# UMich-CURLY/SE3ET

Hardware: AMD Instinct MI355X
Metric: point-cloud pairs/sec (fwd), SE3ET-E 5k-pt pairs (higher is better)
Workload: dtype f32

## Files before the change

se3et_amd/csrc/kpconv_mfma.hip:

```cpp
#include "common.h"
#include "kpconv_sums.h"

namespace {

using namespace kpsum;
using f16x8 = __attribute__((ext_vector_type(8))) _Float16;
using f32x16 = __attribute__((ext_vector_type(16))) float;
using u32x4 = __attribute__((ext_vector_type(4))) unsigned;
using f32x4 = __attribute__((ext_vector_type(4))) float;

#ifndef SE3_KPCONV_STAMP
#define SE3_KPCONV_STAMP(step_, slot_)
#endif
#ifndef SE3_DIAG_WEIGHT_STEP
#define SE3_DIAG_WEIGHT_STEP(gs_, ksp_) (gs_)
#endif

constexpr int kTile4 = kTileB / 16;
constexpr int kHeaderB = 256;

__global__ void kpconv_wmax_kernel(const float* __restrict__ W, int64_t n, unsigned* __restrict__ hdr) {
  float m = 0.f;
  for (int64_t i = (int64_t)blockIdx.x * blockDim.x + threadIdx.x; i < n; i += (int64_t)gridDim.x * blockDim.x) m = fmaxf(m, fabsf(W[i]));
  m = se3_wave_max(m);
  if (se3_lane() == 0) atomicMax(hdr + 1, __float_as_uint(m));
}

__device__ __forceinline__ float weight_scale(unsigned max_bits) {
  const int e = (int)((max_bits >> 23) & 0xff);
  if (e == 0 || e == 0xff) return 1.f;
  return __uint_as_float((unsigned)(127 + 12 - (e - 127)) << 23);
}

__global__ void kpconv_split_weights_f16_kernel(const float* __restrict__ W, int Cin, int Cout, unsigned* __restrict__ hdr,
                                                uint4* __restrict__ Wf) {
  const int NCT = Cout / 32;
  const int64_t frag = blockIdx.x;
  const int ct = (int)(frag % NCT), st = (int)((frag / NCT) % kSteps), cc = (int)(frag / ((int64_t)NCT * kSteps));
  const int lane = threadIdx.x, n = ct * 32 + (lane & 31), u = 2 * st + (lane >> 5);
  const float scale = weight_scale(hdr[1]);
  if (frag == 0 && lane == 0) reinterpret_cast<float*>(hdr)[0] = 1.f / scale;
  f16x8 hi, lo;
#pragma unroll
  for (int j = 0; j < 8; j++) {
    const float w = W[((int64_t)u * Cin + cc * kCC + j) * Cout + n] * scale;
    hi[j] = (_Float16)w;
    lo[j] = (_Float16)(w - (float)hi[j]);
  }
  uint4* dst = Wf + frag * 2 * 64 + lane;
  dst[0] = __builtin_bit_cast(uint4, hi);
  dst[64] = __builtin_bit_cast(uint4, lo);
}

__device__ __forceinline__ int row_point(int i) { return ((i >> 3) << 2) + (i & 3); }
__device__ __forceinline__ int row_rsel(int i) { return (0x96 >> (i >> 2)) & 1; }

template <int NCW, int KS>
__global__ __launch_bounds__(64 * NCW * KS) void kpconv_mfma_kernel(const u32x4* __restrict__ H, const u32x4* __restrict__ Wf,
                                                                    const float* __restrict__ hdr, int64_t P, int64_t tiles, int Cin,
                                                                    int Cout, float* __restrict__ out) {
  constexpr int kThreads = 64 * NCW * KS;
  constexpr int kPF = (kTile4 + kThreads - 1) / kThreads;
  constexpr int kSPW = kSteps / KS;
  static_assert(kSteps % KS == 0, "K split must divide the 18 K16-steps of a chunk");
  extern __shared__ __align__(16) unsigned char lds[];
  unsigned* tab = reinterpret_cast<unsigned*>(lds + kTileB);
  const int tid = threadIdx.x, lane = tid & 63, wave = tid >> 6, cw = wave % NCW, ksp = wave / NCW;
  const int64_t tile = blockIdx.x, p0 = tile * kTP;
  const int NCT = Cout / 32, ct = blockIdx.y * NCW + cw;
  for (int e = tid; e < kSteps * 4; e += kThreads) {
    const int h = e & 1, rsel = (e >> 1) & 1, st = e >> 2;
    const int u = 2 * st + h, s = u / kA, t = u % kA;
    unsigned v = 0;
    for (int rt = 0; rt < 3; rt++) {
      const int r = 2 * rt + rsel;
      v |= (unsigned)run_of(kOrb.id[s][r], kOrb.anchor[t][r]) << (8 * rt);
    }
    tab[e] = v;
  }
  const int i32 = lane & 31, h = lane >> 5;
  const int a_base = row_point(i32) * kRowB;
  const int tab_lane = row_rsel(i32) * 2 + h;
  f32x16 acc[3];
#pragma unroll
  for (int rt = 0; rt < 3; rt++)
#pragma unroll
    for (int v = 0; v < 16; v++) acc[rt][v] = 0.f;
  const int chunks = Cin / kCC;
  u32x4 pf[kPF];
  {
    const u32x4* src = H + tile * kTile4;
#pragma unroll
    for (int i = 0; i < kPF; i++) pf[i] = src[min(tid + i * kThreads, kTile4 - 1)];
  }
  const u32x4* wbase = Wf + (int64_t)ct * 2 * 64 + lane;
  const int64_t wstep = (int64_t)NCT * 2 * 64;
  u32x4 bn0 = wbase[(int64_t)ksp * wstep], bn1 = wbase[(int64_t)ksp * wstep + 64];
  const int64_t last_step = (int64_t)chunks * kSteps - KS + ksp;
  for (int cc = 0; cc < chunks; cc++) {
    __syncthreads();
#pragma unroll
    for (int i = 0; i < kPF; i++)
      if (tid + i * kThreads < kTile4) reinterpret_cast<u32x4*>(lds)[tid + i * kThreads] = pf[i];
    {
      const int cn = cc + 1 < chunks ? cc + 1 : cc;
      const u32x4* src = H + ((int64_t)cn * tiles + tile) * kTile4;
#pragma unroll
      for (int i = 0; i < kPF; i++) pf[i] = src[min(tid + i * kThreads, kTile4 - 1)];
// ... 208 lines not shown
}

constexpr int kStageRow[4] = {0, 392, 836, 1228};
constexpr int kStageDw = 1228 + 384;
template <bool EXT>
__global__ __launch_bounds__(256) void kpconv_orbit_gather_kernel(const float* __restrict__ x, const float* __restrict__ hwt,
                                                                   const int* __restrict__ nbr, const int* __restrict__ cnt, int NNp,
                                                                   int64_t tiles, int Cin, unsigned char* __restrict__ Hs) {
  __shared__ __align__(16) unsigned stage[4][kStageDw];
  const int lane = threadIdx.x & 63, wave = threadIdx.x >> 6, g = lane >> 4, c16 = lane & 15, odd = c16 & 1, half = c16 >> 3;
  const int64_t p = blockIdx.x;
  const int T = blockIdx.y * 4 + wave, chunks = Cin / kCC;
  if (2 * T >= chunks) return;
  const bool has2 = 2 * T + 1 < chunks;
  const unsigned rowlen = (unsigned)(kA * Cin), col = (unsigned)(T * 16 + (has2 || half == 0 ? c16 : c16 - 8));
  const int nv = cnt[p];
  const int* nbrow = nbr + p * NNp;
  const float* hwrow = hwt + p * NNp * 16;
  f32x4 acc[kA];
#pragma unroll
  for (int a = 0; a < kA; a++) acc[a] = f32x4{0.f, 0.f, 0.f, 0.f};
  constexpr int S = EXT ? 40 : 32;
  for (int rd = 0; S * rd < nv; rd++) {
    int nbv[kGN + (EXT ? kGX : 0)];
    GatherOps<EXT> q;
    gather_request_rows<EXT>(nbrow, rd, g, nbv);
    gather_request_ops<EXT, false>(x, hwrow, NNp, rd, g, c16, nbv, rowlen, col, Cin, nv, q);
    gather_multiply<EXT>(q, nv > S * rd + 32, acc);
  }
  unsigned word[kA][4];
  gather_split(acc, odd, word);
  unsigned* st = stage[wave];
  const int cpair = (c16 & 7) >> 1;
#pragma unroll
  for (int a = 0; a < kA; a++)
#pragma unroll
    for (int r = 0; r < 4; r++) st[kStageRow[half * 2 + odd] + (a * 16 + 4 * g + r) * 4 + cpair] = word[a][r];
  for (int e = lane; e < 4 * 96; e += 64) {
    const int row = e / 96, q4 = e - row * 96, hf = row >> 1, piece = row & 1;
    if (hf == 1 && !has2) continue;
    unsigned char* dst = Hs + ((int64_t)(2 * T + hf) * tiles + (p >> 4)) * kTileB + (size_t)piece * kPieceB + (size_t)(p & 15) * kRowB;
    reinterpret_cast<u32x4*>(dst)[q4] = *reinterpret_cast<const u32x4*>(st + kStageRow[row] + q4 * 4);
  }
}

template <int NCW, int KS, int CT, bool EXT, bool BLK>
__global__ __launch_bounds__(64 * (NCW * KS + 8)) void kpconv_fused_kernel(
    const float* __restrict__ x, const float* __restrict__ hwt, const int* __restrict__ nbr, const int* __restrict__ cnt, int NNp,
    const u32x4* __restrict__ Wf, const float* __restrict__ hdr, int64_t P, int Cin, int Cout, float* __restrict__ out,
    float* __restrict__ split_part, int* __restrict__ split_count, const float* __restrict__ x_amax) {
  constexpr int NC = NCW * KS;
  const float xs = x_split_scale(x_amax);
  constexpr int NPW = 8;
  constexpr int kSPW = kSteps / KS;
  static_assert(kSteps % KS == 0, "K split must divide the 18 K16-steps of a chunk");
  extern __shared__ __align__(16) unsigned char lds[];
  unsigned* tab = reinterpret_cast<unsigned*>(lds + 3 * kTileB);
  const int tid = threadIdx.x, lane = tid & 63;
  const int wave = __builtin_amdgcn_readfirstlane(tid >> 6);
  const int64_t tile = blockIdx.x, p0 = tile * kTP;
  const int chunks = Cin / kCC / (int)gridDim.z, chunk0 = blockIdx.z * chunks, pairs = (chunks + 1) / 2;
  for (int e = tid; e < kSteps * 4; e += 64 * (NC + NPW)) {
    const int h = e & 1, rsel = (e >> 1) & 1, st = e >> 2;
    const int u = 2 * st + h, s = u / kA, t = u % kA;
    unsigned v = 0;
    for (int rt = 0; rt < 3; rt++) {
      const int r = 2 * rt + rsel;
      v |= (unsigned)run_of(kOrb.id[s][r], kOrb.anchor[t][r]) << (8 * rt);
    }
    tab[e] = v;
  }
  const int steps_total = chunks + 2;
  if (wave >= NC) {
    const int pw = wave - NC;
    const int g = lane >> 4, c16 = lane & 15, odd = c16 & 1, half = c16 >> 3, cpair = (c16 & 7) >> 1;
    const unsigned rowlen = (unsigned)(kA * Cin);
    const int dst0 = odd * kPieceB + g * 64 + cpair * 4;
    unsigned held[kA][4];
#pragma unroll
    for (int a = 0; a < kA; a++)
#pragma unroll
      for (int r = 0; r < 4; r++) held[a][r] = 0u;
    constexpr int S = EXT ? 40 : 32;
    GatherOps<EXT> ops;
    int nv_cur = 0;
    const int64_t plast = P - 1;
    auto point_of = [&](int u) { return p0 + pw + NPW * (u & 1); };
    auto col_of = [&](int u) {
      const int T = u >> 1;
      return (unsigned)(chunk0 * kCC + T * 16 + ((2 * T + 1 < chunks || half == 0) ? c16 : c16 - 8));
    };
    {
      const int64_t p = point_of(0), pc = p < P ? p : plast;
      int nbv[kGN + (EXT ? kGX : 0)];
      gather_request_rows<EXT>(nbr + pc * NNp, 0, g, nbv);
      nv_cur = p < P ? cnt[pc] : 0;
      gather_request_ops<EXT, BLK>(x, hwt + pc * NNp * 16, NNp, 0, g, c16, nbv, rowlen, col_of(0), Cin, __builtin_amdgcn_readfirstlane(nv_cur), ops);
    }
    for (int u = 0; u < steps_total; u++) {
      SE3_KPCONV_STAMP(u, 0)
      if (u < 2 * pairs) {
        const int T = u >> 1, second = u & 1;
        const int i = pw + NPW * second;
        const int64_t p = p0 + i, pc = p < P ? p : plast;
        const bool has2 = 2 * T + 1 < chunks;
        unsigned char* img_a = lds + ((2 * T) % 3) * kTileB;
        unsigned char* img_b = lds + ((2 * T + 1) % 3) * kTileB;
        if (second && half == 1 && has2) {
// ... 5 lines not shown
        }
        const bool more = u + 1 < 2 * pairs;
        const int64_t pn = point_of(u + 1), pnc = pn < P ? pn : plast;
        int nbn[kGN + (EXT ? kGX : 0)];
        gather_request_rows<EXT>(nbr + pnc * NNp, 0, g, nbn);
        const int nv_next = (more && pn < P) ? cnt[pnc] : 0;
        SE3_KPCONV_STAMP(u, 1)
        f32x4 acc[kA];
#pragma unroll
        for (int a = 0; a < kA; a++) acc[a] = f32x4{0.f, 0.f, 0.f, 0.f};
        const int nv = __builtin_amdgcn_readfirstlane(nv_cur);
        SE3_KPCONV_STAMP(u, 5)
        if (nv > 0) gather_multiply<EXT>(ops, nv > 32, acc, xs);
        SE3_KPCONV_STAMP(u, 6)
        for (int rd = 1; S * rd < nv; rd++) {
          int nbv[kGN + (EXT ? kGX : 0)];
          GatherOps<EXT> q;
          gather_request_rows<EXT>(nbr + pc * NNp, rd, g, nbv);
          gather_request_ops<EXT, BLK>(x, hwt + pc * NNp * 16, NNp, rd, g, c16, nbv, rowlen, col_of(u), Cin, nv, q);
          gather_multiply<EXT>(q, nv > S * rd + 32, acc, xs);
        }
        SE3_KPCONV_STAMP(u, 7)
        gather_request_ops<EXT, BLK>(x, hwt + pnc * NNp * 16, NNp, 0, g, c16, nbn, rowlen, col_of(more ? u + 1 : u), Cin,
                                __builtin_amdgcn_readfirstlane(nv_next), ops);
        nv_cur = nv_next;
        SE3_KPCONV_STAMP(u, 2)
        unsigned word[kA][4];
        gather_split(acc, odd, word);
        unsigned char* dst = (half ? img_b : img_a) + i * kRowB + dst0;
        if (half == 0 || (second && has2)) {
#pragma unroll
          for (int a = 0; a < kA; a++)
#pragma unroll
            for (int r = 0; r < 4; r++) *reinterpret_cast<unsigned*>(dst + (a * 16 + r) * 16) = word[a][r];
        }
#pragma unroll
        for (int a = 0; a < kA; a++)
#pragma unroll
          for (int r = 0; r < 4; r++) held[a][r] = word[a][r];
      }
      SE3_KPCONV_STAMP(u, 3)
      if (u + 1 < steps_total) __syncthreads();
      SE3_KPCONV_STAMP(u, 4)
    }
    if (KS > 1) {
      __syncthreads();
      __syncthreads();
    }
    return;
  }
  const int cw = wave % NCW, ksp = wave / NCW;
  const int NCT = Cout / 32, ct0 = (blockIdx.y * NCW + cw) * CT;
  const int i32 = lane & 31, h = lane >> 5;
  const int a_base = row_point(i32) * kRowB;
  const int tab_lane = row_rsel(i32) * 2 + h;
  f32x16 acc[CT][3];
#pragma unroll
  for (int n = 0; n < CT; n++)
#pragma unroll
    for (int rt = 0; rt < 3; rt++)
#pragma unroll
      for (int v = 0; v < 16; v++) acc[n][rt][v] = 0.f;
  constexpr int BD = (CT == 2 && KS > 1) ? 2 : (CT == 1 ? 6 : 3);
  constexpr int U = BD == 2 ? 2 : 6;
  static_assert(kSPW % U == 0, "K16-steps per wave and chunk must be a multiple of the unroll");
  const int64_t wstep = (int64_t)NCT * 2 * 64;
  const u32x4* wbase = Wf + (int64_t)chunk0 * kSteps * wstep + (int64_t)ct0 * 2 * 64 + lane;
  const int64_t last_step = (int64_t)chunks * kSteps - KS + ksp;
  u32x4 bq[BD][CT][2];
#pragma unroll
  for (int j = 0; j < BD; j++) {
    int64_t gs = ksp + j * KS;
    gs = gs < last_step ? gs : last_step;
#pragma unroll
    for (int n = 0; n < CT; n++) {
      bq[j][n][0] = wbase[gs * wstep + n * 128];
      bq[j][n][1] = wbase[gs * wstep + n * 128 + 64];
    }
  }
  __syncthreads();
  __syncthreads();
  for (int cc = 0; cc < chunks; cc++) {
    const unsigned char* img = lds + (cc % 3) * kTileB;
    SE3_KPCONV_STAMP(cc + 2, 0)
    f16x8 av[2][3][2];
    {
      const unsigned runs = tab[ksp * 4 + tab_lane];
#pragma unroll
      for (int rt = 0; rt < 3; rt++) {
        const int off = a_base + (int)((runs >> (8 * rt)) & 0xff) * 16;
        av[0][rt][0] = *reinterpret_cast<const f16x8*>(img + off);
        av[0][rt][1] = *reinterpret_cast<const f16x8*>(img + off + kPieceB);
      }
    }
#pragma unroll 1
    for (int q0 = 0; q0 < kSPW; q0 += U) {
#pragma unroll
      for (int j = 0; j < U; j++) {
        constexpr int kDummy = 0;
        const int ja = j & 1, jb = j % BD;
        const int st = ksp + (q0 + j) * KS;
        {
          const int sn = st + KS < kSteps ? st + KS : st;
          const unsigned runs = tab[sn * 4 + tab_lane];
#pragma unroll
          for (int rt = 0; rt < 3; rt++) {
            const int off = a_base + (int)((runs >> (8 * rt)) & 0xff) * 16;
            av[ja ^ 1][rt][0] = *reinterpret_cast<const f16x8*>(img + off);
            av[ja ^ 1][rt][1] = *reinterpret_cast<const f16x8*>(img + off + kPieceB);
          }
          if constexpr (CT == 1) __builtin_amdgcn_sched_barrier(0);
        }
#pragma unroll
        for (int n = 0; n < CT; n++) {
          const f16x8 b0 = __builtin_bit_cast(f16x8, bq[jb][n][0]);
#pragma unroll
          for (int rt = 0; rt < 3; rt++) acc[n][rt] = __builtin_amdgcn_mfma_f32_32x32x16_f16(av[ja][rt][1], b0, acc[n][rt], 0, 0, 0);
        }
#pragma unroll
        for (int n = 0; n < CT; n++) {
          const f16x8 b1 = __builtin_bit_cast(f16x8, bq[jb][n][1]);
#pragma unroll
          for (int rt = 0; rt < 3; rt++) acc[n][rt] = __builtin_amdgcn_mfma_f32_32x32x16_f16(av[ja][rt][0], b1, acc[n][rt], 0, 0, 0);
        }
#pragma unroll
        for (int n = 0; n < CT; n++) {
          const f16x8 b0 = __builtin_bit_cast(f16x8, bq[jb][n][0]);
#pragma unroll
          for (int rt = 0; rt < 3; rt++) acc[n][rt] = __builtin_amdgcn_mfma_f32_32x32x16_f16(av[ja][rt][0], b0, acc[n][rt], 0, 0, 0);
        }
        {
          int64_t gs = (int64_t)cc * kSteps + st + BD * KS;
          gs = gs < last_step ? gs : last_step;
          gs = SE3_DIAG_WEIGHT_STEP(gs, ksp);
#pragma unroll
          for (int n = 0; n < CT; n++) {
            bq[jb][n][0] = wbase[gs * wstep + n * 128];
            bq[jb][n][1] = wbase[gs * wstep + n * 128 + 64];
          }
        }
        (void)kDummy;
      }
    }
    SE3_KPCONV_STAMP(cc + 2, 3)
    if (cc + 1 < chunks) __syncthreads();
    SE3_KPCONV_STAMP(cc + 2, 4)
  }
  if (KS > 1) {
    __syncthreads();
    float* red = reinterpret_cast<float*>(lds);
    if (ksp > 0) {
#pragma unroll
      for (int n = 0; n < CT; n++)
#pragma unroll
        for (int rt = 0; rt < 3; rt++)
#pragma unroll
          for (int v = 0; v < 16; v++) red[((((ksp - 1) * NCW + cw) * CT + n) * 48 + rt * 16 + v) * 64 + lane] = acc[n][rt][v];
    }
    __syncthreads();
    if (ksp > 0) return;
#pragma unroll 1
    for (int k = 1; k < KS; k++)
#pragma unroll
      for (int n = 0; n < CT; n++)
#pragma unroll
        for (int rt = 0; rt < 3; rt++)
#pragma unroll
          for (int v = 0; v < 16; v++) acc[n][rt][v] += red[((((k - 1) * NCW + cw) * CT + n) * 48 + rt * 16 + v) * 64 + lane];
  }
  const float inv_scale = hdr[0] / xs;
  const int row_b = Cout * 4;
  const int rows_here = (int)(P - p0 < kTP ? P - p0 : kTP);
  int voff[CT][2];
#pragma unroll
  for (int n = 0; n < CT; n++) {
    voff[n][0] = ((ct0 + n) * 32 + i32) * 4 + h * row_b;
    voff[n][1] = ((ct0 + n) * 32 + i32) * 4 + (1 - h) * row_b;
  }
  constexpr int kAgent = 16;
#pragma unroll
  for (int n = 0; n < CT; n++)
#pragma unroll
    for (int rt = 0; rt < 3; rt++) acc[n][rt] *= inv_scale;
  if (gridDim.z > 1) {
    const int64_t rows_all = (int64_t)gridDim.x * kTP * kA;
    {
      const __amdgpu_buffer_rsrc_t prs =
          __builtin_amdgcn_make_buffer_rsrc(split_part + (blockIdx.z * rows_all + p0 * kA) * Cout, 0, kTP * kA * row_b, 0x00020000);
#pragma unroll
      for (int n = 0; n < CT; n++)
#pragma unroll
        for (int rt = 0; rt < 3; rt++)
#pragma unroll
          for (int v = 0; v < 16; v++) {
            const float val = acc[n][rt][v];
            __builtin_amdgcn_raw_buffer_store_b32(__builtin_bit_cast(unsigned, val), prs, voff[n][(0x6 >> (v >> 2)) & 1],
// ... 258 lines not shown
```

se3et_amd/csrc/kpconv_union.hip:

```cpp
#include "common.h"
#include "kpconv_sums.h"

namespace {

using namespace kpsum;
using f16x8 = __attribute__((ext_vector_type(8))) _Float16;
using f32x16 = __attribute__((ext_vector_type(16))) float;
using u32x4 = __attribute__((ext_vector_type(4))) unsigned;
using f32x4 = __attribute__((ext_vector_type(4))) float;

constexpr int kHeaderB = 256;
#ifndef SE3_UCAP
#define SE3_UCAP 128
#endif
constexpr int kUCap = SE3_UCAP;
constexpr int kKSM = kUCap / 32;
constexpr int kBFragB = 1024;
constexpr int kBImgB = 2 * 3 * kKSM * kBFragB;
constexpr int kScrRow = kUCap + 4;
constexpr int kMaxSub = 16;

__device__ __forceinline__ int row_point(int i) { return ((i >> 3) << 2) + (i & 3); }
__device__ __forceinline__ int row_rsel(int i) { return (0x96 >> (i >> 2)) & 1; }

struct PlanViews {
  int* order;
  int* nsub;
  int4* desc;
  int* urow;
  unsigned char* loc;
};
__host__ __device__ inline size_t align16(size_t v) { return (v + 15) & ~(size_t)15; }
inline PlanViews plan_views(void* plan, int64_t G, int NNp) {
  unsigned char* p = static_cast<unsigned char*>(plan);
  PlanViews v;
  v.order = reinterpret_cast<int*>(p);
  p += align16((size_t)G * 16 * sizeof(int));
  v.nsub = reinterpret_cast<int*>(p);
  p += align16((size_t)G * sizeof(int));
  v.desc = reinterpret_cast<int4*>(p);
  p += (size_t)G * kMaxSub * sizeof(int4);
  v.urow = reinterpret_cast<int*>(p);
  p += align16((size_t)G * 16 * NNp * sizeof(int));
  v.loc = p;
  return v;
}
inline size_t plan_bytes(int64_t G, int NNp) {
  return align16((size_t)G * 16 * sizeof(int)) + align16((size_t)G * sizeof(int)) + (size_t)G * kMaxSub * sizeof(int4) +
         align16((size_t)G * 16 * NNp * sizeof(int)) + align16((size_t)G * 16 * NNp) + 256;
}

struct NeighborTable {
  const float* hwt;
  const int *nbr, *cnt;
  int NNp;
};
NeighborTable table_views(const void* table, int64_t P, int NN) {
  NeighborTable t;
  t.NNp = NN <= 32 ? 32 : (NN + 39) / 40 * 40;
  t.hwt = static_cast<const float*>(table);
  t.nbr = reinterpret_cast<const int*>(t.hwt + (size_t)P * t.NNp * 16);
  t.cnt = t.nbr + (size_t)P * t.NNp;
  return t;
}

__global__ __launch_bounds__(64) void kpconv_union_plan_kernel(const int* __restrict__ nbr, const int* __restrict__ cnt, int NNp,
                                                               const int* __restrict__ order_in, PlanViews pv) {
  __shared__ unsigned long long keys[1024];
  const int lane = threadIdx.x;
  const int64_t group = blockIdx.x;
  const int pid = lane < 16 ? order_in[group * 16 + lane] : -1;
  int c = pid >= 0 ? cnt[pid] : 0;
  c = c < 64 ? c : 64;
  if (lane < 16) pv.order[group * 16 + lane] = pid;
  int off = c;
#pragma unroll
// ... 176 lines not shown
    okeys[i] = k;
  }
  __syncthreads();
  for (int k = 2; k <= n2; k <<= 1)
    for (int j = k >> 1; j > 0; j >>= 1) {
      for (int t = tid; t < (n2 >> 1); t += 1024) {
        const int a = ((t & ~(j - 1)) << 1) | (t & (j - 1)), b = a | j;
        const bool up = (a & k) == 0;
        const unsigned long long x = okeys[a], y = okeys[b];
        if ((x > y) == up) {
          okeys[a] = y;
          okeys[b] = x;
        }
      }
      __syncthreads();
    }
  const int npad = ((n + 15) >> 4) << 4;
  for (int r = tid; r < npad; r += 1024) order[pos0 + r] = r < n ? (int)(start + (int64_t)(okeys[r] & 0xffffu)) : -1;
}

__device__ __forceinline__ void split8(const float (&v)[8], f16x8& hi, f16x8& lo) {
#pragma unroll
  for (int i = 0; i < 8; i++) {
    hi[i] = (_Float16)v[i];
    lo[i] = (_Float16)(v[i] - (float)hi[i]);
  }
}

struct UnionArgs {
  const float* x;
  const float* hwt;
  const int* cnt;
  int NNp;
  const int* order;
  const int* nsub;
  const int4* desc;
  const int* urow;
  const unsigned char* loc;
  const u32x4* Wf;
  const float* hdr;
  int64_t P;
  int64_t G;
  int Cin, Cout;
  float* out;
  float* split_part;
  int* split_count;
  const float* x_amax;
};

template <int NCW, int KS, int CT, bool BLK>
__global__ __launch_bounds__(64 * (NCW * KS + 8)) void kpconv_union_kernel(const UnionArgs a) {
  constexpr int NC = NCW * KS;
  constexpr int NPW = 8;
  constexpr int kSPW = kSteps / KS;
  constexpr bool kIdle = KS > 1;
  static_assert(kSteps % KS == 0, "K split must divide the 18 K16-steps of a chunk");
  static_assert((KS - 1) * NCW * CT * 48 * 64 * 4 <= kTileB, "the K-split partial sums live in one tile image");
  extern __shared__ __align__(16) unsigned char lds[];
  unsigned char* const bimg0 = lds + 2 * kTileB;
  unsigned* tab = reinterpret_cast<unsigned*>(bimg0 + 2 * kBImgB);
  int* pid_s = reinterpret_cast<int*>(tab + kSteps * 4);
  const int tid = threadIdx.x, lane = tid & 63;
  const int wave = __builtin_amdgcn_readfirstlane(tid >> 6);
  const int Cin = a.Cin, Cout = a.Cout, NNp = a.NNp;
  const int64_t G = a.G;
  const int chunks = Cin / kCC / (int)gridDim.z, chunk0 = blockIdx.z * chunks;
  for (int e = tid; e < kSteps * 4; e += 64 * (NC + NPW)) {
    const int h = e & 1, rsel = (e >> 1) & 1, st = e >> 2;
    const int u = 2 * st + h, s = u / kA, t = u % kA;
    unsigned v = 0;
    for (int rt = 0; rt < 3; rt++) {
      const int r = 2 * rt + rsel;
      v |= (unsigned)run_of(kOrb.id[s][r], kOrb.anchor[t][r]) << (8 * rt);
    }
    tab[e] = v;
  }
  __syncthreads();
  if (wave >= NC) {
    const int pw = wave - NC;
    const int g = lane >> 4, col = lane & 15, odd = col & 1, half = col >> 3, cpair = (col & 7) >> 1;
    const unsigned rowlen = (unsigned)(kA * Cin);
    const float xs = x_split_scale(a.x_amax);
    const int task = pw * 60 + lane, oh = task / 12, q = task - oh * 12, oct = oh >> 1, jh = oh & 1;
    const unsigned qoff = BLK ? (unsigned)(q * 4) : (unsigned)((q >> 1) * Cin + (q & 1) * 4);
    const unsigned cstride = BLK ? 48u : 8u;
    const int nt_l = q >> 2, g_l = oct & 3;
    const int bdst = (nt_l * kKSM + (oct >> 2)) * kBFragB + g_l * 256 + jh * 8;
    const int bsw = (nt_l + g_l) & 3;
    float* const scr = reinterpret_cast<float*>(lds + (chunks & 1) * kTileB) + pw * (8 * kScrRow);
    auto meta_load = [&](int64_t grp, int sub) -> int {
      const int* p = lane < 16 ? a.order + grp * 16 + lane
                               : (lane < 20 ? reinterpret_cast<const int*>(a.desc + grp * kMaxSub + sub) + (lane - 16) : a.nsub + grp);
      return lane < 21 ? *p : 0;
    };
    int64_t grp = blockIdx.x;
    int sub = 0, gpar = 0;
    int meta = meta_load(grp, sub);
    unsigned roff[4], roff_n[4];
    int meta2 = 0;
    f32x4 V[4];
#pragma unroll
    for (int j = 0; j < 4; j++) V[j] = f32x4{0.f, 0.f, 0.f, 0.f};
    auto stage_b = [&](int64_t grp_, int meta_, unsigned (&ro)[4]) -> int {
      const int ustart = __builtin_amdgcn_readlane(meta_, 18), ucount = __builtin_amdgcn_readlane(meta_, 19);
      const int* urow = a.urow + grp_ * 16 * NNp + ustart;
      const bool lt = lane < 60 && oct < 4 * ((ucount + 31) >> 5);
#pragma unroll
// ... 101 lines not shown
            if (ks < ksn) {
#pragma unroll
              for (int nt = 0; nt < 3; nt++) {
                const int unit = (col ^ ((nt + g) & 3)) * 16;
                const f16x8 bh = *reinterpret_cast<const f16x8*>(bsrc + (nt * kKSM + ks) * kBFragB + unit);
                const f16x8 bl = *reinterpret_cast<const f16x8*>(bsrc + ((3 + nt) * kKSM + ks) * kBFragB + unit);
                acc[0][nt] = __builtin_amdgcn_mfma_f32_16x16x32_f16(al[0][ks], bh, acc[0][nt], 0, 0, 0);
                acc[1][nt] = __builtin_amdgcn_mfma_f32_16x16x32_f16(al[1][ks], bh, acc[1][nt], 0, 0, 0);
                acc[0][nt] = __builtin_amdgcn_mfma_f32_16x16x32_f16(ah[0][ks], bl, acc[0][nt], 0, 0, 0);
                acc[1][nt] = __builtin_amdgcn_mfma_f32_16x16x32_f16(ah[1][ks], bl, acc[1][nt], 0, 0, 0);
                acc[0][nt] = __builtin_amdgcn_mfma_f32_16x16x32_f16(ah[0][ks], bh, acc[0][nt], 0, 0, 0);
                acc[1][nt] = __builtin_amdgcn_mfma_f32_16x16x32_f16(ah[1][ks], bh, acc[1][nt], 0, 0, 0);
              }
            }
#pragma unroll
          for (int pt = 0; pt < 2; pt++) {
            unsigned char* dst = img + (pw + NPW * pt) * kRowB + odd * kPieceB + cpair * 4 + g * 64;
#pragma unroll
            for (int nt = 0; nt < 3; nt++)
#pragma unroll
              for (int r = 0; r < 4; r++) {
                const float v = acc[pt][nt][r];
                const _Float16 hi = (_Float16)v;
                const _Float16 lo16 = (_Float16)(v - (float)hi);
                const unsigned w = (unsigned)__builtin_bit_cast(unsigned short, hi) | ((unsigned)__builtin_bit_cast(unsigned short, lo16) << 16);
                const unsigned w2 = (unsigned)__builtin_amdgcn_update_dpp(0, (int)w, 0xB1, 0xf, 0xf, false);
                const unsigned word = odd ? ((w2 >> 16) | (w & 0xffff0000u)) : ((w & 0xffffu) | (w2 << 16));
                *reinterpret_cast<unsigned*>(dst + ((2 * nt + half) * 16 + r) * 16) = word;
              }
          }
        }
        if (u == chunks - 1 && has_next) {
          const int ucn = __builtin_amdgcn_readlane(meta_n, 19);
          request(0, lane < 60 && oct < 4 * ((ucn + 31) >> 5), roff_n);
        }
        __syncthreads();
      }
      if (!has_next) break;
      if (last_sub) gpar ^= 1;
      grp = ngrp;
      sub = nsubi;
      meta = meta_n;
      meta2 = meta2_n;
#pragma unroll
      for (int j = 0; j < 4; j++) roff[j] = roff_n[j];
    }
    __syncthreads();
    if (kIdle) __syncthreads();
    return;
  }
  const int cw = wave % NCW, ksp = wave / NCW;
  const int NCT = Cout / 32, ct0 = (blockIdx.y * NCW + cw) * CT;
  const int i32 = lane & 31, h = lane >> 5;
  const int a_base = row_point(i32) * kRowB;
  const int tab_lane = row_rsel(i32) * 2 + h;
  f32x16 acc[CT][3];
#pragma unroll
  for (int n = 0; n < CT; n++)
#pragma unroll
    for (int rt = 0; rt < 3; rt++)
#pragma unroll
      for (int v = 0; v < 16; v++) acc[n][rt][v] = 0.f;
  constexpr int BD = (CT == 2 && KS > 1) ? 2 : (CT == 1 ? 6 : 3);
  constexpr int U = BD == 2 ? 2 : 6;
  static_assert(kSPW % U == 0, "K16-steps per wave and chunk must be a multiple of the unroll");
  const int64_t wstep = (int64_t)NCT * 2 * 64;
  const u32x4* wbase = a.Wf + (int64_t)chunk0 * kSteps * wstep + (int64_t)ct0 * 2 * 64 + lane;
  const int total_steps = chunks * kSteps;
  u32x4 bq[BD][CT][2];
#pragma unroll
  for (int j = 0; j < BD; j++) {
    int gs = ksp + j * KS;
    gs = gs < total_steps ? gs : gs - total_steps;
#pragma unroll
    for (int n = 0; n < CT; n++) {
      bq[j][n][0] = wbase[gs * wstep + n * 128];
      bq[j][n][1] = wbase[gs * wstep + n * 128 + 64];
    }
  }
  constexpr int kAgent = 16;
  auto contract = [&](int cc) {
    const unsigned char* img = lds + (cc & 1) * kTileB;
    f16x8 av[2][3][2];
    {
      const unsigned runs = tab[ksp * 4 + tab_lane];
#pragma unroll
      for (int rt = 0; rt < 3; rt++) {
        const int off = a_base + (int)((runs >> (8 * rt)) & 0xff) * 16;
        av[0][rt][0] = *reinterpret_cast<const f16x8*>(img + off);
        av[0][rt][1] = *reinterpret_cast<const f16x8*>(img + off + kPieceB);
      }
    }
#pragma unroll 1
    for (int q0 = 0; q0 < kSPW; q0 += U) {
#pragma unroll
      for (int j = 0; j < U; j++) {
        const int ja = j & 1, jb = j % BD;
        const int st = ksp + (q0 + j) * KS;
        {
          const int sn = st + KS < kSteps ? st + KS : st;
          const unsigned runs = tab[sn * 4 + tab_lane];
#pragma unroll
          for (int rt = 0; rt < 3; rt++) {
            const int off = a_base + (int)((runs >> (8 * rt)) & 0xff) * 16;
            av[ja ^ 1][rt][0] = *reinterpret_cast<const f16x8*>(img + off);
            av[ja ^ 1][rt][1] = *reinterpret_cast<const f16x8*>(img + off + kPieceB);
          }
          if constexpr (CT == 1) __builtin_amdgcn_sched_barrier(0);
        }
#pragma unroll
        for (int n = 0; n < CT; n++) {
          const f16x8 b0 = __builtin_bit_cast(f16x8, bq[jb][n][0]);
#pragma unroll
          for (int rt = 0; rt < 3; rt++) acc[n][rt] = __builtin_amdgcn_mfma_f32_32x32x16_f16(av[ja][rt][1], b0, acc[n][rt], 0, 0, 0);
        }
#pragma unroll
        for (int n = 0; n < CT; n++) {
          const f16x8 b1 = __builtin_bit_cast(f16x8, bq[jb][n][1]);
#pragma unroll
          for (int rt = 0; rt < 3; rt++) acc[n][rt] = __builtin_amdgcn_mfma_f32_32x32x16_f16(av[ja][rt][0], b1, acc[n][rt], 0, 0, 0);
        }
#pragma unroll
        for (int n = 0; n < CT; n++) {
          const f16x8 b0 = __builtin_bit_cast(f16x8, bq[jb][n][0]);
#pragma unroll
          for (int rt = 0; rt < 3; rt++) acc[n][rt] = __builtin_amdgcn_mfma_f32_32x32x16_f16(av[ja][rt][0], b0, acc[n][rt], 0, 0, 0);
        }
        {
          int gs = cc * kSteps + st + BD * KS;
          gs = gs < total_steps ? gs : gs - total_steps;
#pragma unroll
          for (int n = 0; n < CT; n++) {
            bq[jb][n][0] = wbase[gs * wstep + n * 128];
            bq[jb][n][1] = wbase[gs * wstep + n * 128 + 64];
          }
        }
      }
    }
  };
  auto epilogue = [&](int64_t group, int par) {
    const float inv_scale = a.hdr[0] / x_split_scale(a.x_amax);
    const int row_b = Cout * 4;
    int voff[CT][2];
#pragma unroll
    for (int n = 0; n < CT; n++) {
      voff[n][0] = ((ct0 + n) * 32 + i32) * 4 + h * row_b;
      voff[n][1] = ((ct0 + n) * 32 + i32) * 4 + (1 - h) * row_b;
    }
#pragma unroll
    for (int n = 0; n < CT; n++)
#pragma unroll
      for (int rt = 0; rt < 3; rt++) acc[n][rt] *= inv_scale;
    bool owner = true;
    if (gridDim.z > 1) {
      const int64_t rows_all = G * kTP * kA;
      {
        const __amdgpu_buffer_rsrc_t prs =
            __builtin_amdgcn_make_buffer_rsrc(a.split_part + (blockIdx.z * rows_all + group * kTP * kA) * Cout, 0, kTP * kA * row_b, 0x00020000);
#pragma unroll
        for (int n = 0; n < CT; n++)
#pragma unroll
          for (int rt = 0; rt < 3; rt++)
#pragma unroll
            for (int v = 0; v < 16; v++) {
              const float val = acc[n][rt][v];
              __builtin_amdgcn_raw_buffer_store_b32(__builtin_bit_cast(unsigned, val), prs, voff[n][(0x6 >> (v >> 2)) & 1],
                                                    (v * kA + 2 * rt) * row_b, kAgent);
            }
      }
      asm volatile("s_waitcnt vmcnt(0)" ::: "memory");
      int* counter = a.split_count + group * (NCT / CT) + ct0 / CT;
      int ticket = 0;
      if (lane == 0) ticket = __hip_atomic_fetch_add(counter, 1, __ATOMIC_RELAXED, __HIP_MEMORY_SCOPE_AGENT);
      ticket = __builtin_amdgcn_readfirstlane(ticket);
      owner = ticket == (int)gridDim.z - 1;
      if (owner) {
        if (lane == 0) __hip_atomic_store(counter, 0, __ATOMIC_RELAXED, __HIP_MEMORY_SCOPE_AGENT);
#pragma unroll
        for (int n = 0; n < CT; n++)
#pragma unroll
          for (int rt = 0; rt < 3; rt++)
#pragma unroll
            for (int v = 0; v < 16; v++) acc[n][rt][v] = 0.f;
#pragma unroll 1
        for (int z = 0; z < (int)gridDim.z; z++) {
          const __amdgpu_buffer_rsrc_t prs =
              __builtin_amdgcn_make_buffer_rsrc(a.split_part + (z * rows_all + group * kTP * kA) * Cout, 0, kTP * kA * row_b, 0x00020000);
#pragma unroll
          for (int n = 0; n < CT; n++)
#pragma unroll
            for (int rt = 0; rt < 3; rt++)
#pragma unroll
              for (int v = 0; v < 16; v++)
                acc[n][rt][v] += __builtin_bit_cast(float, __builtin_amdgcn_raw_buffer_load_b32(prs, voff[n][(0x6 >> (v >> 2)) & 1],
                                                                                                (v * kA + 2 * rt) * row_b, kAgent));
        }
      }
    }
    if (owner) {
#pragma unroll
      for (int v = 0; v < 16; v++) {
        const int pid = __builtin_amdgcn_readfirstlane(pid_s[par * 16 + v]);
        if (pid < 0) continue;
        const __amdgpu_buffer_rsrc_t ors = __builtin_amdgcn_make_buffer_rsrc(a.out + (int64_t)pid * kA * Cout, 0, kA * row_b, 0x00020000);
#pragma unroll
        for (int n = 0; n < CT; n++)
#pragma unroll
          for (int rt = 0; rt < 3; rt++) {
            const float val = acc[n][rt][v];
            __builtin_amdgcn_raw_buffer_store_b32(__builtin_bit_cast(unsigned, val), ors, voff[n][(0x6 >> (v >> 2)) & 1], 2 * rt * row_b, 0);
          }
      }
    }
  };
  float* const red = reinterpret_cast<float*>(lds + kTileB);
  int64_t grp = blockIdx.x, prev_grp = 0;
  int sub = 0, par = 0, prev_par = 0;
  int nsub = grp < G ? a.nsub[grp] : 0;
  bool prev_last = false;
  __syncthreads();
  if (kIdle) __syncthreads();
  for (;;) {
    if (prev_last) {
      if (ksp == 0) {
        if (KS > 1) {
#pragma unroll 1
          for (int kk = 1; kk < KS; kk++)
#pragma unroll
            for (int n = 0; n < CT; n++)
#pragma unroll
              for (int rt = 0; rt < 3; rt++)
#pragma unroll
                for (int v = 0; v < 16; v++) acc[n][rt][v] += red[((((kk - 1) * NCW + cw) * CT + n) * 48 + rt * 16 + v) * 64 + lane];
        }
        epilogue(prev_grp, prev_par);
      }
#pragma unroll
      for (int n = 0; n < CT; n++)
#pragma unroll
        for (int rt = 0; rt < 3; rt++)
#pragma unroll
          for (int v = 0; v < 16; v++) acc[n][rt][v] = 0.f;
    }
    if (grp >= G) break;
    __syncthreads();
#pragma unroll 1
    for (int cc = 0; cc < chunks; cc++) {
      contract(cc);
      __syncthreads();
    }
    prev_last = sub + 1 >= nsub;
    prev_grp = grp;
    prev_par = par;
    if (kIdle) {
      if (prev_last && ksp > 0) {
#pragma unroll
        for (int n = 0; n < CT; n++)
#pragma unroll
          for (int rt = 0; rt < 3; rt++)
#pragma unroll
            for (int v = 0; v < 16; v++) red[((((ksp - 1) * NCW + cw) * CT + n) * 48 + rt * 16 + v) * 64 + lane] = acc[n][rt][v];
      }
      __syncthreads();
    }
    if (prev_last) {
      grp += gridDim.x;
      sub = 0;
      par ^= 1;
      nsub = grp < G ? a.nsub[grp] : 0;
    } else {
      sub++;
    }
  }
// ... 217 lines not shown
```

Baseline: 460.6.

## Share a restructured MFMA consumer loop with piece-split LDS prefetch across kernels

Pulls the per-chunk MFMA contraction loop of the fused and union KPConv kernels into a shared ConsumerLoop template. The run-table lookups are now carried in registers (r0/r1) across steps and chunks instead of being reread before each load. For CT=2 the two A pieces are loaded separately and interleaved with MFMA groups behind sched barriers, and the weight buffer depth for that case drops from 3 to 2. The goal is fewer live A-fragment registers and better overlap of LDS reads with MFMAs. The cost is a more fragile schedule and tighter index wraparound logic.

```diff
diff --git a/se3et_amd/csrc/kpconv_consumer.h b/se3et_amd/csrc/kpconv_consumer.h
--- /dev/null
+++ b/se3et_amd/csrc/kpconv_consumer.h
@@ -0,0 +1,120 @@
+#pragma once
+#include "kpconv_sums.h"
+
+#ifndef SE3_DIAG_WEIGHT_STEP
+#define SE3_DIAG_WEIGHT_STEP(gs_, ksp_) (gs_)
+#endif
+
+namespace kpsum {
+
+using f16x8 = __attribute__((ext_vector_type(8))) _Float16;
+using f32x16 = __attribute__((ext_vector_type(16))) float;
+using u32x4 = __attribute__((ext_vector_type(4))) unsigned;
+
+__device__ __forceinline__ int row_point(int i) { return ((i >> 3) << 2) + (i & 3); }
+__device__ __forceinline__ int row_rsel(int i) { return (0x96 >> (i >> 2)) & 1; }
+
+template <int KS, int CT>
+struct ConsumerLoop {
+  static_assert(CT == 1 || CT == 2, "one or two column tiles per wave");
+  static_assert(kSteps % KS == 0, "K split must divide the 18 K16-steps of a chunk");
+  static constexpr int kSPW = kSteps / KS;
+  static constexpr int BD = CT == 1 ? 6 : 2;
+  static constexpr int U = BD;
+  static_assert(kSPW % U == 0, "K16-steps per wave and chunk must be a multiple of the unroll");
+  static constexpr int kSeq = CT == 1 ? kSPW + 1 : kSPW;
+
+  static __device__ __forceinline__ unsigned entry(const unsigned* tab, int tab_lane, int idx) {
+    idx = idx >= kSeq ? idx - kSeq : idx;
+    idx = idx < kSPW ? idx : kSPW - 1;
+    return tab[tab_lane + idx * (KS * 4)];
+  }
+  static __device__ __forceinline__ void lane_rows(int ksp, int& a_base, int& tab_lane) {
+    int lane = (int)__builtin_amdgcn_mbcnt_hi(~0u, __builtin_amdgcn_mbcnt_lo(~0u, 0u));
+    asm volatile("" : "+v"(lane));
+    const int i32 = lane & 31, h = lane >> 5;
+    a_base = row_point(i32) * kRowB;
+    tab_lane = ksp * 4 + row_rsel(i32) * 2 + h;
+  }
+  static __device__ __forceinline__ void start(const unsigned* tab, int ksp, unsigned& r0, unsigned& r1) {
+    int a_base, tab_lane;
+    lane_rows(ksp, a_base, tab_lane);
+    r0 = entry(tab, tab_lane, 0);
+    r1 = CT == 1 ? entry(tab, tab_lane, 1) : 0u;
+  }
+  template <int PIECE>
+  static __device__ __forceinline__ void read_piece(const unsigned char* img, int a_base, unsigned runs, f16x8 (&av)[3][2]) {
+#pragma unroll
+    for (int rt = 0; rt < 3; rt++) {
+      const int off = a_base + (int)((runs >> (8 * rt)) & 0xff) * 16;
+      av[rt][PIECE] = *reinterpret_cast<const f16x8*>(img + off + PIECE * kPieceB);
+    }
+  }
+  template <int PA, int PB>
+  static __device__ __forceinline__ void group(const f16x8 (&av)[3][2], const u32x4 (&b)[CT][2], f32x16 (&acc)[CT][3]) {
+#pragma unroll
+    for (int n = 0; n < CT; n++) {
+      const f16x8 bp = __builtin_bit_cast(f16x8, b[n][PB]);
+#pragma unroll
+      for (int rt = 0; rt < 3; rt++) acc[n][rt] = __builtin_amdgcn_mfma_f32_32x32x16_f16(av[rt][PA], bp, acc[n][rt], 0, 0, 0);
+    }
+  }
+
+  template <class WeightStep>
+  static __device__ __forceinline__ void chunk(const unsigned char* img, const unsigned* tab, unsigned& r0, unsigned& r1,
+                                               const u32x4* wbase, int64_t wstep, int ksp, WeightStep weight_step, u32x4 (&bq)[BD][CT][2],
+                                               f32x16 (&acc)[CT][3]) {
+    int a_base, tab_lane;
+    lane_rows(ksp, a_base, tab_lane);
+    f16x8 av[CT == 1 ? 2 : 1][3][2];
+    if constexpr (CT == 1) {
+      read_piece<0>(img, a_base, r0, av[0]);
+      read_piece<1>(img, a_base, r0, av[0]);
+      r0 = r1;
+      r1 = entry(tab, tab_lane, 2);
+    } else {
+      read_piece<1>(img, a_base, r0, av[0]);
+    }
+    auto refill = [&](int slot, int s) {
+      const auto gs = weight_step(ksp + s * KS);
+#pragma unroll
+      for (int n = 0; n < CT; n++) {
+        bq[slot][n][0] = wbase[gs * wstep + n * 128];
+        bq[slot][n][1] = wbase[gs * wstep + n * 128 + 64];
+      }
+    };
+#pragma unroll 1
+    for (int q0 = 0; q0 < kSPW; q0 += U) {
+#pragma unroll
+      for (int j = 0; j < U; j++) {
+        const int jb = j % BD, q = q0 + j;
+        if constexpr (CT == 1) {
+          const int ja = j & 1;
+          read_piece<0>(img, a_base, r0, av[ja ^ 1]);
+          read_piece<1>(img, a_base, r0, av[ja ^ 1]);
+          r0 = r1;
+          r1 = entry(tab, tab_lane, q + 3);
+          __builtin_amdgcn_sched_barrier(0);
+          group<1, 0>(av[ja], bq[jb], acc);
+          group<0, 1>(av[ja], bq[jb], acc);
+          group<0, 0>(av[ja], bq[jb], acc);
+          refill(jb, q + BD);
+        } else {
+          read_piece<0>(img, a_base, r0, av[0]);
+          r0 = entry(tab, tab_lane, q + 1);
+          __builtin_amdgcn_sched_barrier(0);
+          group<1, 0>(av[0], bq[jb], acc);
+          __builtin_amdgcn_sched_barrier(0);
+          read_piece<1>(img, a_base, r0, av[0]);
+          __builtin_amdgcn_sched_barrier(0);
+          group<0, 1>(av[0], bq[jb], acc);
+          group<0, 0>(av[0], bq[jb], acc);
+          refill(jb, q + BD);
+          __builtin_amdgcn_sched_barrier(0);
+        }
+      }
+    }
+  }
+};
+
+}
diff --git a/se3et_amd/csrc/kpconv_mfma.hip b/se3et_amd/csrc/kpconv_mfma.hip
--- a/se3et_amd/csrc/kpconv_mfma.hip
+++ b/se3et_amd/csrc/kpconv_mfma.hip
@@ -1,19 +1,14 @@
 #include "common.h"
 #include "kpconv_sums.h"
+#include "kpconv_consumer.h"
 
 namespace {
 
 using namespace kpsum;
-using f16x8 = __attribute__((ext_vector_type(8))) _Float16;
-using f32x16 = __attribute__((ext_vector_type(16))) float;
-using u32x4 = __attribute__((ext_vector_type(4))) unsigned;
 using f32x4 = __attribute__((ext_vector_type(4))) float;
 
 #ifndef SE3_KPCONV_STAMP
 #define SE3_KPCONV_STAMP(step_, slot_)
-#endif
-#ifndef SE3_DIAG_WEIGHT_STEP
-#define SE3_DIAG_WEIGHT_STEP(gs_, ksp_) (gs_)
 #endif
 
 constexpr int kTile4 = kTileB / 16;
@@ -51,9 +46,6 @@
   dst[0] = __builtin_bit_cast(uint4, hi);
   dst[64] = __builtin_bit_cast(uint4, lo);
 }
-
-__device__ __forceinline__ int row_point(int i) { return ((i >> 3) << 2) + (i & 3); }
-__device__ __forceinline__ int row_rsel(int i) { return (0x96 >> (i >> 2)) & 1; }
 
 template <int NCW, int KS>
 __global__ __launch_bounds__(64 * NCW * KS) void kpconv_mfma_kernel(const u32x4* __restrict__ H, const u32x4* __restrict__ Wf,
@@ -368,8 +360,6 @@
   constexpr int NC = NCW * KS;
   const float xs = x_split_scale(x_amax);
   constexpr int NPW = 8;
-  constexpr int kSPW = kSteps / KS;
-  static_assert(kSteps % KS == 0, "K split must divide the 18 K16-steps of a chunk");
   extern __shared__ __align__(16) unsigned char lds[];
   unsigned* tab = reinterpret_cast<unsigned*>(lds + 3 * kTileB);
   const int tid = threadIdx.x, lane = tid & 63;
@@ -481,8 +471,6 @@
   const int cw = wave % NCW, ksp = wave / NCW;
   const int NCT = Cout / 32, ct0 = (blockIdx.y * NCW + cw) * CT;
   const int i32 = lane & 31, h = lane >> 5;
-  const int a_base = row_point(i32) * kRowB;
-  const int tab_lane = row_rsel(i32) * 2 + h;
   f32x16 acc[CT][3];
 #pragma unroll
   for (int n = 0; n < CT; n++)
@@ -490,9 +478,8 @@
     for (int rt = 0; rt < 3; rt++)
 #pragma unroll
       for (int v = 0; v < 16; v++) acc[n][rt][v] = 0.f;
-  constexpr int BD = (CT == 2 && KS > 1) ? 2 : (CT == 1 ? 6 : 3);
-  constexpr int U = BD == 2 ? 2 : 6;
-  static_assert(kSPW % U == 0, "K16-steps per wave and chunk must be a multiple of the unroll");
+  using Loop = ConsumerLoop<KS, CT>;
+  constexpr int BD = Loop::BD;
   const int64_t wstep = (int64_t)NCT * 2 * 64;
   const u32x4* wbase = Wf + (int64_t)chunk0 * kSteps * wstep + (int64_t)ct0 * 2 * 64 + lane;
   const int64_t last_step = (int64_t)chunks * kSteps - KS + ksp;
@@ -508,69 +495,18 @@
     }
   }
   __syncthreads();
+  unsigned r0, r1;
+  Loop::start(tab, ksp, r0, r1);
   __syncthreads();
   for (int cc = 0; cc < chunks; cc++) {
-    const unsigned char* img = lds + (cc % 3) * kTileB;
     SE3_KPCONV_STAMP(cc + 2, 0)
-    f16x8 av[2][3][2];
-    {
-      const unsigned runs = tab[ksp * 4 + tab_lane];
-#pragma unroll
-      for (int rt = 0; rt < 3; rt++) {
-        const int off = a_base + (int)((runs >> (8 * rt)) & 0xff) * 16;
-        av[0][rt][0] = *reinterpret_cast<const f16x8*>(img + off);
-        av[0][rt][1] = *reinterpret_cast<const f16x8*>(img + off + kPieceB);
-      }
-    }
-#pragma unroll 1
-    for (int q0 = 0; q0 < kSPW; q0 += U) {
-#pragma unroll
-      for (int j = 0; j < U; j++) {
-        constexpr int kDummy = 0;
-        const int ja = j & 1, jb = j % BD;
-        const int st = ksp + (q0 + j) * KS;
-        {
-          const int sn = st + KS < kSteps ? st + KS : st;
-          const unsigned runs = tab[sn * 4 + tab_lane];
-#pragma unroll
-          for (int rt = 0; rt < 3; rt++) {
-            const int off = a_base + (int)((runs >> (8 * rt)) & 0xff) * 16;
-            av[ja ^ 1][rt][0] = *reinterpret_cast<const f16x8*>(img + off);
-            av[ja ^ 1][rt][1] = *reinterpret_cast<const f16x8*>(img + off + kPieceB);
-          }
-          if constexpr (CT == 1) __builtin_amdgcn_sched_barrier(0);
-        }
-#pragma unroll
-        for (int n = 0; n < CT; n++) {
-          const f16x8 b0 = __builtin_bit_cast(f16x8, bq[jb][n][0]);
-#pragma unroll
-          for (int rt = 0; rt < 3; rt++) acc[n][rt] = __builtin_amdgcn_mfma_f32_32x32x16_f16(av[ja][rt][1], b0, acc[n][rt], 0, 0, 0);
-        }
-#pragma unroll
-        for (int n = 0; n < CT; n++) {
-          const f16x8 b1 = __builtin_bit_cast(f16x8, bq[jb][n][1]);
-#pragma unroll
-          for (int rt = 0; rt < 3; rt++) acc[n][rt] = __builtin_amdgcn_mfma_f32_32x32x16_f16(av[ja][rt][0], b1, acc[n][rt], 0, 0, 0);
-        }
-#pragma unroll
-        for (int n = 0; n < CT; n++) {
-          const f16x8 b0 = __builtin_bit_cast(f16x8, bq[jb][n][0]);
-#pragma unroll
-          for (int rt = 0; rt < 3; rt++) acc[n][rt] = __builtin_amdgcn_mfma_f32_32x32x16_f16(av[ja][rt][0], b0, acc[n][rt], 0, 0, 0);
-        }
-        {
-          int64_t gs = (int64_t)cc * kSteps + st + BD * KS;
-          gs = gs < last_step ? gs : last_step;
-          gs = SE3_DIAG_WEIGHT_STEP(gs, ksp);
-#pragma unroll
-          for (int n = 0; n < CT; n++) {
-            bq[jb][n][0] = wbase[gs * wstep + n * 128];
-            bq[jb][n][1] = wbase[gs * wstep + n * 128 + 64];
-          }
-        }
-        (void)kDummy;
-      }
-    }
+    Loop::chunk(lds + (cc % 3) * kTileB, tab, r0, r1, wbase, wstep, ksp,
+                [&](int s) {
+                  int64_t gs = (int64_t)cc * kSteps + s;
+                  gs = gs < last_step ? gs : last_step;
+                  return (int64_t)SE3_DIAG_WEIGHT_STEP(gs, ksp);
+                },
+                bq, acc);
     SE3_KPCONV_STAMP(cc + 2, 3)
     if (cc + 1 < chunks) __syncthreads();
     SE3_KPCONV_STAMP(cc + 2, 4)
diff --git a/se3et_amd/csrc/kpconv_union.hip b/se3et_amd/csrc/kpconv_union.hip
--- a/se3et_amd/csrc/kpconv_union.hip
+++ b/se3et_amd/csrc/kpconv_union.hip
@@ -1,12 +1,10 @@
 #include "common.h"
 #include "kpconv_sums.h"
+#include "kpconv_consumer.h"
 
 namespace {
 
 using namespace kpsum;
-using f16x8 = __attribute__((ext_vector_type(8))) _Float16;
-using f32x16 = __attribute__((ext_vector_type(16))) float;
-using u32x4 = __attribute__((ext_vector_type(4))) unsigned;
 using f32x4 = __attribute__((ext_vector_type(4))) float;
 
 constexpr int kHeaderB = 256;
@@ -19,9 +17,6 @@
 constexpr int kBImgB = 2 * 3 * kKSM * kBFragB;
 constexpr int kScrRow = kUCap + 4;
 constexpr int kMaxSub = 16;
-
-__device__ __forceinline__ int row_point(int i) { return ((i >> 3) << 2) + (i & 3); }
-__device__ __forceinline__ int row_rsel(int i) { return (0x96 >> (i >> 2)) & 1; }
 
 struct PlanViews {
   int* order;
@@ -304,7 +299,6 @@
 __global__ __launch_bounds__(64 * (NCW * KS + 8)) void kpconv_union_kernel(const UnionArgs a) {
   constexpr int NC = NCW * KS;
   constexpr int NPW = 8;
-  constexpr int kSPW = kSteps / KS;
   constexpr bool kIdle = KS > 1;
   static_assert(kSteps % KS == 0, "K split must divide the 18 K16-steps of a chunk");
   static_assert((KS - 1) * NCW * CT * 48 * 64 * 4 <= kTileB, "the K-split partial sums live in one tile image");
@@ -512,8 +506,6 @@
   const int cw = wave % NCW, ksp = wave / NCW;
   const int NCT = Cout / 32, ct0 = (blockIdx.y * NCW + cw) * CT;
   const int i32 = lane & 31, h = lane >> 5;
-  const int a_base = row_point(i32) * kRowB;
-  const int tab_lane = row_rsel(i32) * 2 + h;
   f32x16 acc[CT][3];
 #pragma unroll
   for (int n = 0; n < CT; n++)
@@ -521,9 +513,8 @@
     for (int rt = 0; rt < 3; rt++)
 #pragma unroll
       for (int v = 0; v < 16; v++) acc[n][rt][v] = 0.f;
-  constexpr int BD = (CT == 2 && KS > 1) ? 2 : (CT == 1 ? 6 : 3);
-  constexpr int U = BD == 2 ? 2 : 6;
-  static_assert(kSPW % U == 0, "K16-steps per wave and chunk must be a multiple of the unroll");
+  using Loop = ConsumerLoop<KS, CT>;
+  constexpr int BD = Loop::BD;
   const int64_t wstep = (int64_t)NCT * 2 * 64;
   const u32x4* wbase = a.Wf + (int64_t)chunk0 * kSteps * wstep + (int64_t)ct0 * 2 * 64 + lane;
   const int total_steps = chunks * kSteps;
@@ -539,64 +530,14 @@
     }
   }
   constexpr int kAgent = 16;
+  unsigned r0 = 0, r1 = 0;
   auto contract = [&](int cc) {
-    const unsigned char* img = lds + (cc & 1) * kTileB;
-    f16x8 av[2][3][2];
-    {
-      const unsigned runs = tab[ksp * 4 + tab_lane];
-#pragma unroll
-      for (int rt = 0; rt < 3; rt++) {
-        const int off = a_base + (int)((runs >> (8 * rt)) & 0xff) * 16;
-        av[0][rt][0] = *reinterpret_cast<const f16x8*>(img + off);
-        av[0][rt][1] = *reinterpret_cast<const f16x8*>(img + off + kPieceB);
-      }
-    }
-#pragma unroll 1
-    for (int q0 = 0; q0 < kSPW; q0 += U) {
-#pragma unroll
-      for (int j = 0; j < U; j++) {
-        const int ja = j & 1, jb = j % BD;
-        const int st = ksp + (q0 + j) * KS;
-        {
-          const int sn = st + KS < kSteps ? st + KS : st;
-          const unsigned runs = tab[sn * 4 + tab_lane];
-#pragma unroll
-          for (int rt = 0; rt < 3; rt++) {
-            const int off = a_base + (int)((runs >> (8 * rt)) & 0xff) * 16;
-            av[ja ^ 1][rt][0] = *reinterpret_cast<const f16x8*>(img + off);
-            av[ja ^ 1][rt][1] = *reinterpret_cast<const f16x8*>(img + off + kPieceB);
-          }
-          if constexpr (CT == 1) __builtin_amdgcn_sched_barrier(0);
-        }
-#pragma unroll
-        for (int n = 0; n < CT; n++) {
-          const f16x8 b0 = __builtin_bit_cast(f16x8, bq[jb][n][0]);
-#pragma unroll
-          for (int rt = 0; rt < 3; rt++) acc[n][rt] = __builtin_amdgcn_mfma_f32_32x32x16_f16(av[ja][rt][1], b0, acc[n][rt], 0, 0, 0);
-        }
-#pragma unroll
-        for (int n = 0; n < CT; n++) {
-          const f16x8 b1 = __builtin_bit_cast(f16x8, bq[jb][n][1]);
-#pragma unroll
-          for (int rt = 0; rt < 3; rt++) acc[n][rt] = __builtin_amdgcn_mfma_f32_32x32x16_f16(av[ja][rt][0], b1, acc[n][rt], 0, 0, 0);
-        }
-#pragma unroll
-        for (int n = 0; n < CT; n++) {
-          const f16x8 b0 = __builtin_bit_cast(f16x8, bq[jb][n][0]);
-#pragma unroll
-          for (int rt = 0; rt < 3; rt++) acc[n][rt] = __builtin_amdgcn_mfma_f32_32x32x16_f16(av[ja][rt][0], b0, acc[n][rt], 0, 0, 0);
-        }
-        {
-          int gs = cc * kSteps + st + BD * KS;
-          gs = gs < total_steps ? gs : gs - total_steps;
-#pragma unroll
-          for (int n = 0; n < CT; n++) {
-            bq[jb][n][0] = wbase[gs * wstep + n * 128];
-            bq[jb][n][1] = wbase[gs * wstep + n * 128 + 64];
-          }
-        }
-      }
-    }
+    Loop::chunk(lds + (cc & 1) * kTileB, tab, r0, r1, wbase, wstep, ksp,
+                [&](int s) {
+                  const int gs = cc * kSteps + s;
+                  return gs < total_steps ? gs : gs - total_steps;
+                },
+                bq, acc);
   };
   auto epilogue = [&](int64_t group, int par) {
     const float inv_scale = a.hdr[0] / x_split_scale(a.x_amax);
@@ -679,6 +620,7 @@
   int nsub = grp < G ? a.nsub[grp] : 0;
   bool prev_last = false;
   __syncthreads();
+  Loop::start(tab, ksp, r0, r1);
   if (kIdle) __syncthreads();
   for (;;) {
     if (prev_last) {
```

After: 463.8, median of 4. About the same (+0.7%).
